# bifurcationkit/BifurcationKit.jl

Hardware: NVIDIA H100
Metric: continuation steps/sec (SH2d PALC) (higher is better)
Workload: dtype f64

## Files before the change

### bifurcationkit.jl_b200/csrc/bk_common.cuh

```cuda
#pragma once
#include <cuda_runtime.h>
#include <stdint.h>
#include <stdlib.h>
#include <string>
#include <unordered_map>
#include <vector>
#include "../../include/bk200.h"
#include <nvtx3/nvToolsExt.h>

struct BkRange {
  explicit BkRange(const char* name) { nvtxRangePushA(name); }
  ~BkRange() { nvtxRangePop(); }
};

#define BK_MAX_PAR 8
#define BK_NSM_FALLBACK 132

struct OpDesc {
  int kind;
  int nx, ny, nz;
  double cx, cy, cz;
  double par[BK_MAX_PAR];
  const double* u;
  double a0, a1;
  long long N;
  int bordered;
  const double* ba;
  const double* bb;
  double bc, bshift, bscale;
  const double* ba2;
  const double* bb2;
  double bc01, bc10, bc11;
  const double* phi;
  const double* fcache;
  int cplx;
  double a0i;
  int transpose;
};

namespace bkg {
#define BKG_MAXPASS 16
struct Plan {
  int n;
  int L;
  int npass;
  int radix[BKG_MAXPASS];
  const double2* wl;
  const double2* ph;
  double dst_scale;
};
}

enum { PW_NONE = 0, PW_RESID = 1, PW_JVP = 2, PW_FLEFT = 3, PW_FRIGHT = 4 };
struct PerPw {
  int pro;
  int epi;
  const double* v;
  const double* u;
  const double* sp;
  double a0, a1, l, nu;
  double spc;
};
#define PW_D 1

struct Precond {
  int kind = BK_PC_NONE;
  double a0 = 0, a1 = 0;
  double* lam[3] = {nullptr, nullptr, nullptr};
  int ttype[3] = {0, 0, 0};
  int fast[3] = {0, 0, 0};
  double2* ftw[3] = {nullptr, nullptr, nullptr};
  double2* fom[3] = {nullptr, nullptr, nullptr};
  double2* flam2[3] = {nullptr, nullptr, nullptr};
  bkg::Plan gplan[3] = {};
  double2* gwl[3] = {nullptr, nullptr, nullptr};
  double2* gph[3] = {nullptr, nullptr, nullptr};
  double* work = nullptr;
  double* work2 = nullptr;
  double* tri = nullptr;
  double2* tdft = nullptr;
  double po_r = 0, po_nu = 0, po_T = 0;
};

struct BkKindTraits {
  int ndims;
  int fields;
  int extra;
  bool jac_sym;
  bool has_jt;
  bool complex_ok;
  bool pow2_grid;
  bool has_jets;
};
const BkKindTraits* bk_kind_traits(int kind);

struct BkEventTimer {
  std::vector<std::pair<cudaEvent_t, cudaEvent_t>> pairs;
  size_t used = 0;
  void begin(cudaStream_t st) {
    if (used == pairs.size()) {
      cudaEvent_t a, b;
      cudaEventCreate(&a);
      cudaEventCreate(&b);
      pairs.push_back({a, b});
    }
    cudaEventRecord(pairs[used++].first, st);
  }
  void end(cudaStream_t st) { cudaEventRecord(pairs[used - 1].second, st); }
  long long harvest(double& ms) {
    long long k = 0;
    for (size_t i = 0; i < used; ++i) {
      float t = 0;
      if (cudaEventElapsedTime(&t, pairs[i].first, pairs[i].second) == cudaSuccess) {
        ms += t;
        ++k;
      }
    }
    used = 0;
    return k;
  }
  void destroy() {
    for (auto& p : pairs) {
      cudaEventDestroy(p.first);
      cudaEventDestroy(p.second);
    }
    pairs.clear();
    used = 0;
  }
};

struct bk_ctx {
  int device = 0;
  int nsm = BK_NSM_FALLBACK;
  cudaStream_t stream = nullptr;
  int kind = 0;
  long long dims[3] = {1, 1, 1};
  double lengths[3] = {1, 1, 1};
  double par[BK_MAX_PAR] = {0};
  long long N = 0;
  long long N0 = 0;
  bool cplx = false;
  double shift_imag = 0;
  bool transpose = false;
  int m = 0;
  long long ld = 0;
  double* u_state = nullptr;
  double jpar[BK_MAX_PAR] = {0};
  bool have_state = false;
  double* phi = nullptr;
  double* xpi = nullptr;
  double* fcache = nullptr;
  double phi_dot_xpi = 0;
  double* V = nullptr;
  double* w = nullptr;
  double* z = nullptr;
  double* r = nullptr;
  double* scales = nullptr;
  double* gcoef = nullptr;
  double* hcols = nullptr;
  double* hcols2 = nullptr;
  double* h_pinned = nullptr;
  double* partials = nullptr;
  int gmax = 0;
  unsigned int* counters = nullptr;
  double* red_out = nullptr;
  double* red_pinned = nullptr;
  double* coef_pinned = nullptr;
  std::vector<cudaEvent_t> events;
  std::vector<double*> stage;
  double* host_pinned = nullptr;
  std::vector<double*> tmp;
  double* mom_stage = nullptr;
  size_t mom_stage_cap = 0;
  void* mom_work = nullptr;
  size_t mom_work_cap = 0;
  std::unordered_map<double*, size_t> vec_live;
  std::vector<std::pair<size_t, double*>> vec_pool;
  double* Q = nullptr;
  double* Q2 = nullptr;
  int q2cap = 0;
  int qcap = 0;
  double* eig_dev = nullptr;
  double* eig_pinned = nullptr;
  Precond pc;
  bk_stats stats = {};
  bool timing = false;
  int timing_every = 1;
  long long solve_count = 0;
  bool timing_now = false;
  BkEventTimer fused_timer;
  BkEventTimer pc_timer;
  std::unordered_map<const void*, size_t> smem_attr;
  std::string err;
};

int bk_fail(bk_ctx* c, int code, const char* what, const char* file, int line);
#define BK_CUDA(c, expr)                                                             \
  do {                                                                               \
    cudaError_t _e = (expr);                                                         \
    if (_e != cudaSuccess) return bk_fail((c), BK_ERR_CUDA, cudaGetErrorString(_e), __FILE__, __LINE__); \
  } while (0)
#define BK_CHECK(c, cond, msg)                                                       \
  do {                                                                               \
    if (!(cond)) return bk_fail((c), BK_ERR_ARG, (msg), __FILE__, __LINE__);         \
  } while (0)
#define BK_ENTER(c)                                 \
  do {                                              \
    if (!(c)) return BK_ERR_ARG;                    \
    if (cudaSetDevice((c)->device) != cudaSuccess)  \
      return bk_fail((c), BK_ERR_CUDA, "cudaSetDevice failed", __FILE__, __LINE__); \
  } while (0)
#define BK_TRY(expr)                 \
  do {                               \
    int _s = (expr);                 \
    if (_s < 0) return _s;           \
  } while (0)

static inline int bk_lin_grid(const bk_ctx* c, long long n) {
  long long g = (n + 255) / 256;
  long long cap = (long long)c->nsm * 8;
  return (int)(g < cap ? (g > 0 ? g : 1) : cap);
}
static inline int bk_reduce_grid(const bk_ctx* c, long long n) {
  const int g = bk_lin_grid(c, n);
  return g < c->gmax ? g : c->gmax;
}
static inline double bk_inv_h2(const bk_ctx* c, int d) {
  const double h = 2 * c->lengths[d] / c->dims[d];
  return 1.0 / (h * h);
}

bool bk_is_device_ptr(const void* p);
int bk_stage_in(bk_ctx* c, const double* p, long long n, int slot, bool copy_in, double** dev);
int bk_stage_out(bk_ctx* c, double* p, long long n, const double* dev);

OpDesc bk_make_op(bk_ctx* c, double a0, double a1);
OpDesc bk_make_residual_op(bk_ctx* c);
int bk_launch_residual(bk_ctx* c, const double* u_dev, double* out_dev);
int bk_launch_apply(bk_ctx* c, const OpDesc& op, const double* in_dev, const double* in_scale_ptr, double* out_dev);
int bk_potrap_refresh_cache(bk_ctx* c);

int bk_precond_apply_dev(bk_ctx* c, const double* in_dev, double* out_dev, long long n);

int bk_periodic_setup(bk_ctx* c);
int bk_periodic_residual(bk_ctx* c, const OpDesc& op, const double* u, double* out);
int bk_periodic_jvp(bk_ctx* c, const OpDesc& op, const double* in, const double* sp, double* out);
int bk_periodic_fused(bk_ctx* c, const OpDesc& op, const double* in, const double* sp, double* out, bool left);

int bk_dev_axpby(bk_ctx* c, double* y, double a, const double* x, double b, long long n);
int bk_dev_scale(bk_ctx* c, double* x, double a, long long n);
int bk_dev_dot(bk_ctx* c, const double* x, const double* y, long long n, double* out_host);
int bk_dev_norminf(bk_ctx* c, const double* x, long long n, double* out_host);
int bk_dev_copy(bk_ctx* c, double* dst, const double* src, long long n);

int bk_gmres_dev(bk_ctx* c, const OpDesc& op, const double* rhs_dev, double* x_dev, const bk_gmres_opts* o,
                 int* converged, int* iters, double* resnorm);
int bk_launch_dots(bk_ctx* c, const double* basis, const double* scales, const double* w, long long n, int j, double* hcol,
                   double* gcoef);
int bk_launch_update(bk_ctx* c, const double* basis, const double* gcoef, const double* w, long long n, int j, double* vout,
                     double* h_out, double* scale_out);
int bk_launch_lincomb(bk_ctx* c, const double* basis, const double* scales, double* x, double beta, long long n, int k,
                      const double* coef_dev);
int bk_tmp(bk_ctx* c, int slot, double** out);

void bk_grant_smem(int device, const void* kern, size_t bytes);
template <typename K>
static inline void bk_ensure_smem(bk_ctx* c, K kern, size_t bytes) {
  size_t& cur = c->smem_attr[(const void*)kern];
  if (bytes > cur) {
    bk_grant_smem(c->device, (const void*)kern, bytes);
    cur = bytes;
  }
}

#ifdef __CUDACC__
template <typename... KArgs, typename... Args>
static inline cudaError_t bk_launch_pdl(void (*kern)(KArgs...), dim3 grid, dim3 block, size_t smem, cudaStream_t st, bool pdl,
                                        Args&&... args) {
  cudaLaunchConfig_t cfg = {};
  cfg.gridDim = grid;
  cfg.blockDim = block;
  cfg.dynamicSmemBytes = smem;
  cfg.stream = st;
  cudaLaunchAttribute at[1];
  at[0].id = cudaLaunchAttributeProgrammaticStreamSerialization;
  at[0].val.programmaticStreamSerializationAllowed = 1;
  cfg.attrs = at;
  static int no_pdl = -1;
  if (no_pdl < 0) no_pdl = getenv("BK_NO_PDL") ? 1 : 0;
  cfg.numAttrs = pdl && !no_pdl ? 1 : 0;
  return cudaLaunchKernelEx(&cfg, kern, KArgs(args)...);
}
template <typename... KArgs, typename... Args>
static inline int bk_launch_ex(bk_ctx* c, bool pdl, void (*kern)(KArgs...), dim3 grid, dim3 block, size_t smem,
                               Args&&... args) {
  if (smem) bk_ensure_smem(c, kern, smem);
  bk_launch_pdl(kern, grid, block, smem, c->stream, pdl, static_cast<Args&&>(args)...);
  BK_CUDA(c, cudaGetLastError());
  c->stats.kernel_launches++;
  return BK_OK;
}
template <typename... KArgs, typename... Args>
static inline int bk_launch(bk_ctx* c, void (*kern)(KArgs...), dim3 grid, dim3 block, size_t smem, Args&&... args) {
  return bk_launch_ex(c, true, kern, grid, block, smem, static_cast<Args&&>(args)...);
}
template <typename... KArgs, typename... Args>
static inline int bk_launch_ordered(bk_ctx* c, void (*kern)(KArgs...), dim3 grid, dim3 block, size_t smem, Args&&... args) {
  return bk_launch_ex(c, false, kern, grid, block, smem, static_cast<Args&&>(args)...);
}
__device__ __forceinline__ void bk_pdl_sync() {
  asm volatile("griddepcontrol.wait;" ::: "memory");
  asm volatile("griddepcontrol.launch_dependents;" ::: "memory");
}
#endif

#ifdef __CUDACC__
__device__ __forceinline__ double bk_warp_sum(double v) {
#pragma unroll
  for (int o = 16; o > 0; o >>= 1) v += __shfl_xor_sync(0xffffffffu, v, o);
  return v;
}
__device__ __forceinline__ double bk_nanmax(double a, double b) { return (a != a) ? a : ((b != b) ? b : fmax(a, b)); }
__device__ __forceinline__ double bk_warp_max(double v) {
#pragma unroll
  for (int o = 16; o > 0; o >>= 1) v = bk_nanmax(v, __shfl_xor_sync(0xffffffffu, v, o));
  return v;
}
__device__ __forceinline__ bool bk_last_block(unsigned int* counter, int* s_flag) {
  __threadfence();
  __syncthreads();
  if (threadIdx.x == 0) {
    unsigned int t = atomicAdd(counter, 1u);
    int last = (t == gridDim.x * gridDim.y * gridDim.z - 1);
    if (last) *counter = 0u;
    *s_flag = last;
  }
  __syncthreads();
  bool last = (*s_flag != 0);
  if (last) __threadfence();
  return last;
}
template <bool MAX>
__device__ __forceinline__ double bk_red(double a, double b) { return MAX ? bk_nanmax(a, b) : a + b; }
template <int K, bool MAX = false>
__device__ __forceinline__ bool bk_grid_reduce(double (&v)[K], double* __restrict__ partials, unsigned int* counter) {
  __shared__ double s_w[K][8];
  __shared__ int s_flag;
  const int lane = threadIdx.x & 31, wid = threadIdx.x >> 5;
#pragma unroll
  for (int k = 0; k < K; ++k) {
    const double t = MAX ? bk_warp_max(v[k]) : bk_warp_sum(v[k]);
    if (lane == 0) s_w[k][wid] = t;
  }
  __syncthreads();
  if (threadIdx.x < K) {
    double t = 0.0;
    for (int w = 0; w < 8; ++w) t = bk_red<MAX>(t, s_w[threadIdx.x][w]);
    partials[(size_t)threadIdx.x * gridDim.x + blockIdx.x] = t;
  }
  if (!bk_last_block(counter, &s_flag)) return false;
  double t[K];
#pragma unroll
  for (int k = 0; k < K; ++k) t[k] = 0.0;
  for (int i = threadIdx.x; i < (int)gridDim.x; i += blockDim.x)
#pragma unroll
    for (int k = 0; k < K; ++k) t[k] = bk_red<MAX>(t[k], __ldcg(partials + (size_t)k * gridDim.x + i));
#pragma unroll
  for (int k = 0; k < K; ++k) {
    t[k] = MAX ? bk_warp_max(t[k]) : bk_warp_sum(t[k]);
    if (lane == 0) s_w[k][wid] = t[k];
  }
  __syncthreads();
  if (threadIdx.x != 0) return false;
#pragma unroll
  for (int k = 0; k < K; ++k) {
    v[k] = 0.0;
    for (int w = 0; w < 8; ++w) v[k] = bk_red<MAX>(v[k], s_w[k][w]);
  }
  return true;
}
#endif
```

### bifurcationkit.jl_b200/csrc/bk_precond.cu

```cuda
#include <cmath>
#include <cstdlib>
#include <utility>
#include <vector>
#include "bk_common.cuh"

#include "bk_fft_fast.cuh"
#include "bk_fft_gen.cuh"

static __global__ void __launch_bounds__(256) k_sh_symbol_div(double* __restrict__ a, int nx, int ny, int nz,
                                                              const double* __restrict__ lx, const double* __restrict__ ly,
                                                              const double* __restrict__ lz, double shift, double scale) {
  const long long total = (long long)nx * ny * nz;
  for (long long q = (long long)blockIdx.x * blockDim.x + threadIdx.x; q < total; q += (long long)gridDim.x * blockDim.x) {
    int i = (int)(q % nx), j = (int)((q / nx) % ny), k = (int)(q / ((long long)nx * ny));
    double t = 1.0 + lx[i] + ly[j] + (lz ? lz[k] : 0.0);
    a[q] = a[q] * scale / (t * t + shift);
  }
}
static __global__ void __launch_bounds__(256) k_helmholtz_symbol_div(double* __restrict__ a, int nx, int ny, long long nblocks,
                                                                     const double* __restrict__ lx,
                                                                     const double* __restrict__ ly, double a0, double a1) {
  const long long n = (long long)nx * ny, total = n * nblocks;
  for (long long q = (long long)blockIdx.x * blockDim.x + threadIdx.x; q < total; q += (long long)gridDim.x * blockDim.x) {
    long long g = q % n;
    int i = (int)(g % nx), j = (int)(g / nx);
    a[q] = a[q] / (a0 + a1 * (lx[i] + ly[j]));
  }
}

#define BK_PO_KMAX 64
static __global__ void __launch_bounds__(128) k_potrap_time(double* __restrict__ B, long long n, int nx, int K,
                                                            const double* __restrict__ lamx, const double* __restrict__ lamy,
                                                            double h, double r, double nu, const double2* __restrict__ tw) {
  const long long g = (long long)blockIdx.x * blockDim.x + threadIdx.x;
  if (g >= n) return;
  const double lam = lamx[g % nx] + lamy[g / nx];
  double2 wp[BK_PO_KMAX], wm[BK_PO_KMAX];
  for (int i = 0; i < K; ++i) {
    const double a = B[(long long)(2 * i) * n + g], b = B[(long long)(2 * i + 1) * n + g];
    wp[i] = make_double2(a, b);
    wm[i] = make_double2(a, -b);
  }
  double2 yp[BK_PO_KMAX], ym[BK_PO_KMAX];
  const double invK = 1.0 / K;
  for (int k = 0; k < K; ++k) {
    double2 ap = make_double2(0, 0), am = make_double2(0, 0);
    int idx = 0;
    for (int i = 0; i < K; ++i) {
      const double2 t = tw[idx];
      ap.x += wp[i].x * t.x - wp[i].y * t.y;
      ap.y += wp[i].x * t.y + wp[i].y * t.x;
      am.x += wm[i].x * t.x - wm[i].y * t.y;
      am.y += wm[i].x * t.y + wm[i].y * t.x;
      idx += k;
      if (idx >= K) idx -= K;
    }
    const double2 gk = tw[k];
    const double2 omg = make_double2(1.0 - gk.x, -gk.y), opg = make_double2(1.0 + gk.x, gk.y);
    const double cr = lam + r;
    double2 sp = make_double2(omg.x - 0.5 * h * (opg.x * cr - opg.y * nu), omg.y - 0.5 * h * (opg.x * nu + opg.y * cr));
    double2 sm = make_double2(omg.x - 0.5 * h * (opg.x * cr + opg.y * nu), omg.y - 0.5 * h * (-opg.x * nu + opg.y * cr));
    const double dp = 1.0 / (sp.x * sp.x + sp.y * sp.y), dm = 1.0 / (sm.x * sm.x + sm.y * sm.y);
    yp[k] = make_double2((ap.x * sp.x + ap.y * sp.y) * dp * invK, (ap.y * sp.x - ap.x * sp.y) * dp * invK);
    ym[k] = make_double2((am.x * sm.x + am.y * sm.y) * dm * invK, (am.y * sm.x - am.x * sm.y) * dm * invK);
  }
  for (int i = 0; i < K; ++i) {
    double2 ap = make_double2(0, 0), am = make_double2(0, 0);
    int idx = 0;
    for (int k = 0; k < K; ++k) {
      const double2 t = tw[idx];
      ap.x += yp[k].x * t.x + yp[k].y * t.y;
      ap.y += yp[k].y * t.x - yp[k].x * t.y;
      am.x += ym[k].x * t.x + ym[k].y * t.y;
      am.y += ym[k].y * t.x - ym[k].x * t.y;
      idx += i;
      if (idx >= K) idx -= K;
    }
    B[(long long)(2 * i) * n + g] = 0.5 * (ap.x + am.x);
    B[(long long)(2 * i + 1) * n + g] = 0.5 * (ap.y - am.y);
  }
}
static __global__ void __launch_bounds__(128) k_potrap_time_tr(double* __restrict__ B, long long n, int nx, int K,
                                                               const double* __restrict__ lamx, const double* __restrict__ lamy,
                                                               double h, double r, double nu, const double2* __restrict__ tw) {
  const long long g = (long long)blockIdx.x * blockDim.x + threadIdx.x;
  if (g >= n) return;
  const double lam = lamx[g % nx] + lamy[g / nx];
  double2 wp[BK_PO_KMAX], wm[BK_PO_KMAX];
  for (int i = 0; i < K; ++i) {
    double a = B[(long long)(2 * i) * n + g], b = B[(long long)(2 * i + 1) * n + g];
    if (i == 0) {
      a += B[(long long)(2 * K) * n + g];
      b += B[(long long)(2 * K + 1) * n + g];
    }
    wp[i] = make_double2(a, b);
    wm[i] = make_double2(a, -b);
  }
  double2 yp[BK_PO_KMAX], ym[BK_PO_KMAX];
  const double invK = 1.0 / K;
  for (int k = 0; k < K; ++k) {
    double2 ap = make_double2(0, 0), am = make_double2(0, 0);
    int idx = 0;
    for (int i = 0; i < K; ++i) {
      const double2 t = tw[idx];
      ap.x += wp[i].x * t.x - wp[i].y * t.y;
      ap.y += wp[i].x * t.y + wp[i].y * t.x;
      am.x += wm[i].x * t.x - wm[i].y * t.y;
      am.y += wm[i].x * t.y + wm[i].y * t.x;
      idx += k;
      if (idx >= K) idx -= K;
    }
    const double2 gk = tw[k];
    const double2 omg = make_double2(1.0 - gk.x, -gk.y), opg = make_double2(1.0 + gk.x, gk.y);
    const double cr = lam + r;
    double2 sp = make_double2(omg.x - 0.5 * h * (opg.x * cr - opg.y * nu), omg.y - 0.5 * h * (opg.x * nu + opg.y * cr));
    double2 sm = make_double2(omg.x - 0.5 * h * (opg.x * cr + opg.y * nu), omg.y - 0.5 * h * (-opg.x * nu + opg.y * cr));
    sp.y = -sp.y;
    sm.y = -sm.y;
    const double dp = 1.0 / (sp.x * sp.x + sp.y * sp.y), dm = 1.0 / (sm.x * sm.x + sm.y * sm.y);
    yp[k] = make_double2((ap.x * sp.x + ap.y * sp.y) * dp * invK, (ap.y * sp.x - ap.x * sp.y) * dp * invK);
    ym[k] = make_double2((am.x * sm.x + am.y * sm.y) * dm * invK, (am.y * sm.x - am.x * sm.y) * dm * invK);
  }
  for (int i = 0; i < K; ++i) {
    double2 ap = make_double2(0, 0), am = make_double2(0, 0);
    int idx = 0;
    for (int k = 0; k < K; ++k) {
      const double2 t = tw[idx];
      ap.x += yp[k].x * t.x + yp[k].y * t.y;
      ap.y += yp[k].y * t.x - yp[k].x * t.y;
      am.x += ym[k].x * t.x + ym[k].y * t.y;
      am.y += ym[k].y * t.x - ym[k].x * t.y;
      idx += i;
      if (idx >= K) idx -= K;
    }
    B[(long long)(2 * i) * n + g] = 0.5 * (ap.x + am.x);
    B[(long long)(2 * i + 1) * n + g] = 0.5 * (ap.y - am.y);
  }
}
static __global__ void __launch_bounds__(256) k_potrap_close(const double* __restrict__ in, double* __restrict__ out,
                                                             long long Ns, int M) {
  const long long i = (long long)blockIdx.x * blockDim.x + threadIdx.x;
  if (i < Ns) out[(long long)(M - 1) * Ns + i] = in[(long long)(M - 1) * Ns + i] + out[i];
  if (i == 0) out[(long long)M * Ns] = in[(long long)M * Ns];
}

static __global__ void k_thomas(const double* __restrict__ tri, const double* __restrict__ in, double* __restrict__ out, int n) {
  if (blockIdx.x != 0 || threadIdx.x != 0) return;
  const double* cp = tri;
  const double* di = tri + n;
  const double* lo = tri + 2 * n;
  double prev = in[0] * di[0];
  out[0] = prev;
  for (int i = 1; i < n; ++i) {
    prev = (in[i] - lo[i] * prev) * di[i];
    out[i] = prev;
  }
  for (int i = n - 2; i >= 0; --i) out[i] -= cp[i] * out[i + 1];
}

static int upload(bk_ctx* c, void** dst, const void* src, size_t bytes) {
  if (*dst) cudaFree(*dst);
  *dst = nullptr;
  BK_CUDA(c, cudaMalloc(dst, bytes));
  BK_CUDA(c, cudaMemcpy(*dst, src, bytes, cudaMemcpyHostToDevice));
  return BK_OK;
}

static int fast_loge(long long n) {
  static int e = -1;
  if (e < 0) {
    const char* a = getenv("BK_FFT_LOGE");
    e = a ? atoi(a) : 0;
    if (e < 2 || e > 5) e = 0;
  }
  if (e) return e;
  return n >= 1024 ? 3 : 2;
}
static int fast_logn(long long n) {
  static int off = -1;
  if (off < 0) off = getenv("BK_FFT_NO_FAST") ? 1 : 0;
  if (off) return 0;
  for (int l = fast_loge(n) + 1; l <= 11; ++l)
    if (l >= 6 && n == (1LL << l)) return l;
  return 0;
}
#define BKF_DISPATCH_N(LE, LOGN, ...)                                                   \
  switch (LOGN) {                                                                      \
    case 6: { using FC = bkf::Cfg<6, LE>; __VA_ARGS__; } break;                        \
    case 7: { using FC = bkf::Cfg<7, LE>; __VA_ARGS__; } break;                        \
    case 8: { using FC = bkf::Cfg<8, LE>; __VA_ARGS__; } break;                        \
    case 9: { using FC = bkf::Cfg<9, LE>; __VA_ARGS__; } break;                        \
    case 10: { using FC = bkf::Cfg<10, LE>; __VA_ARGS__; } break;                      \
    default: { using FC = bkf::Cfg<11, LE>; __VA_ARGS__; } break;                      \
  }
#define BKF_DISPATCH(LOGN, ...)                                                        \
  switch (fast_loge(1LL << (LOGN))) {                                                               \
    case 2: BKF_DISPATCH_N(2, LOGN, __VA_ARGS__) break;                                \
    case 3: BKF_DISPATCH_N(3, LOGN, __VA_ARGS__) break;                                \
    case 4: BKF_DISPATCH_N(4, LOGN, __VA_ARGS__) break;                                \
    default: BKF_DISPATCH_N(5, LOGN, __VA_ARGS__) break;                               \
  }

template <class FC>
static int fast_setup(bk_ctx* c, int d, const double* lam_host) {
  std::vector<double> tw, om, lam2;
  bkf::build_tables<FC>(tw, om, lam2, lam_host);
  Precond& pc = c->pc;
  if (tw.empty()) tw.assign(2, 0.0);
  BK_TRY(upload(c, (void**)&pc.ftw[d], tw.data(), 8 * tw.size()));
  BK_TRY(upload(c, (void**)&pc.fom[d], om.data(), 8 * om.size()));
  BK_TRY(upload(c, (void**)&pc.flam2[d], lam2.data(), 8 * lam2.size()));
  return BK_OK;
}

template <class FC>
static int fast_launch(bk_ctx* c, int d, bool strided, int mode, const double* in, double* out, const bkf::Geom& g,
                       const bkf::Symbol* sy, const PerPw* pw = nullptr) {
  Precond& pc = c->pc;
  bkf::Tables tb{pc.ftw[d], pc.fom[d], pc.flam2[d]};
  bkf::Symbol s0{};
  if (sy) s0 = *sy;
  PerPw p0{};
  if (pw) p0 = *pw;
  if (strided) {
    static decltype(&bkf::k_strided<FC, 0>) const kern[4] = {bkf::k_strided<FC, 0>, bkf::k_strided<FC, 1>, bkf::k_strided<FC, 2>,
                                                             bkf::k_strided<FC, 3>};
    const dim3 grid((g.nb + 2 * FC::PP - 1) / (2 * FC::PP), g.nouter);
    return bk_launch(c, kern[mode], grid, dim3(FC::THREADS), mode >= 2 ? FC::SMEM_FUSED : FC::SMEM, in, out, g, tb, s0);
  }
  static decltype(&bkf::k_contig<FC, 0>) const kern[4] = {bkf::k_contig<FC, 0>, bkf::k_contig<FC, 1>, bkf::k_contig<FC, 2>,
                                                          bkf::k_contig<FC, 3>};
  const dim3 grid((unsigned)((g.nb + 2 * FC::PP - 1) / (2 * FC::PP)));
  return bk_launch(c, kern[mode], grid, dim3(FC::THREADS), FC::SMEM, in, out, g, tb, p0);
}

static void factorize(int L, bkg::Plan& pl) {
  pl.npass = 0;
  while (L % 4 == 0 && pl.npass < BKG_MAXPASS) {
    pl.radix[pl.npass++] = 4;
    L /= 4;
  }
  for (int p = 2; L > 1 && pl.npass < BKG_MAXPASS; ++p)
    while (L % p == 0 && pl.npass < BKG_MAXPASS) {
      pl.radix[pl.npass++] = p;
      L /= p;
    }
}
#define BKG_THREADS 512
#define BKG_SMEM_BUDGET (100 * 1024)
#define BKG_SMEM_MAX (200 * 1024)
static int gen_ppg(int L) {
  long long per = 32LL * L;
  int p = (int)(BKG_SMEM_BUDGET / per);
  if (p < 1) p = 1;
  if (p > 8) p = 8;
  return p;
}

static int gen_setup(bk_ctx* c, int d, int n, int type) {
  Precond& pc = c->pc;
  bkg::Plan& pl = pc.gplan[d];
  pl.n = n;
  pl.L = type == 0 ? 2 * n : 2 * n + 2;
  BK_CHECK(c, 32LL * pl.L <= BKG_SMEM_MAX, "line too long for the general transform kernel (n <= 3199)");
  factorize(pl.L, pl);
  const long double PI = 3.14159265358979323846264338327950288L;
  std::vector<double> wl(2 * (size_t)pl.L), ph(2 * (size_t)n);
  for (int t = 0; t < pl.L; ++t) {
    wl[2 * t] = (double)cosl(-2.0L * PI * t / pl.L);
    wl[2 * t + 1] = (double)sinl(-2.0L * PI * t / pl.L);
  }
  for (int k = 0; k < n; ++k) {
    ph[2 * k] = (double)cosl(-PI * k / (2.0L * n));
    ph[2 * k + 1] = (double)sinl(-PI * k / (2.0L * n));
  }
  BK_TRY(upload(c, (void**)&pc.gwl[d], wl.data(), 8 * wl.size()));
  BK_TRY(upload(c, (void**)&pc.gph[d], ph.data(), 8 * ph.size()));
  pl.wl = pc.gwl[d];
  pl.ph = pc.gph[d];
  pl.dst_scale = 0.5 * sqrt(2.0 / (n + 1.0));
  return BK_OK;
}

static int gen_launch(bk_ctx* c, int d, bool strided, int mode, const double* in, double* out, const bkf::Geom& g) {
  const bkg::Plan& pl = c->pc.gplan[d];
  const int ppg = gen_ppg(pl.L);
  const size_t sm = 32 * (size_t)pl.L * ppg;
  const long long npairs = ((long long)g.nb + 1) / 2;
  dim3 grid((unsigned)((npairs + ppg - 1) / ppg), strided ? g.nouter : 1);
  static decltype(&bkg::k_gen<false, 0>) const kern[2][3] = {{bkg::k_gen<false, 0>, bkg::k_gen<false, 1>, bkg::k_gen<false, 2>},
                                                              {bkg::k_gen<true, 0>, bkg::k_gen<true, 1>, bkg::k_gen<true, 2>}};
  return bk_launch(c, kern[strided][mode], grid, dim3(BKG_THREADS), sm, in, out, g, pl, ppg);
}

static int setup_dim(bk_ctx* c, int d, long long n, double inv_h2, int type, bool even_nx) {
  Precond& pc = c->pc;
  std::vector<double> lam(n);
  const long double PI = 3.14159265358979323846264338327950288L;
  for (long long k = 0; k < n; ++k)
    lam[k] = (type == 0) ? (double)((2.0L * cosl(PI * k / n) - 2.0L)) * inv_h2
                         : (double)(-(2.0L - 2.0L * cosl(PI * (k + 1) / (n + 1)))) * inv_h2;
  BK_TRY(upload(c, (void**)&pc.lam[d], lam.data(), 8 * n));
  pc.ttype[d] = type;
  pc.fast[d] = (type == 0 && even_nx) ? fast_logn(n) : 0;
  if (pc.fast[d]) {
    BKF_DISPATCH(pc.fast[d], BK_TRY(fast_setup<FC>(c, d, lam.data())));
  }
  return gen_setup(c, d, (int)n, type);
}

int bk_periodic_setup(bk_ctx* c) {
  Precond& pc = c->pc;
  const long double PI = 3.14159265358979323846264338327950288L;
  for (int d = 0; d < 2; ++d) {
    const long long n = c->dims[d];
    int logn = 0;
    while ((1LL << logn) < n) ++logn;
    std::vector<double> lam(n);
    for (long long k = 0; k < n; ++k) {
      const long double ks = (long double)(k <= n / 2 ? k : k - n), w = PI * ks / (long double)c->lengths[d];
      lam[k] = (double)(-w * w);
    }
    BK_TRY(upload(c, (void**)&pc.lam[d], lam.data(), 8 * n));
    pc.fast[d] = logn;
    BKF_DISPATCH(logn, BK_TRY(fast_setup<FC>(c, d, lam.data())));
  }
  if (!pc.work) BK_CUDA(c, cudaMalloc(&pc.work, 8 * (size_t)c->ld));
  if (!pc.work2) BK_CUDA(c, cudaMalloc(&pc.work2, 8 * (size_t)c->ld));
  return BK_OK;
}

static int periodic_pipeline(bk_ctx* c, const double* in, double* out, const PerPw& pw, bool neg, double gain, double shift,
                             const double* tail_src = nullptr, double* tail_dst = nullptr, int tail_n = 0) {
  Precond& pc = c->pc;
  const int nx = (int)c->dims[0], ny = (int)c->dims[1];
  const bkf::Geom gx{1, nx, ny, 1}, gy{nx, (long long)nx * ny, nx, 1};
  const bkf::Symbol sy{pc.lam[0], nullptr, shift, gain / ((double)nx * (double)ny), tail_src, tail_dst, tail_n, neg ? 1 : 0};
  BKF_DISPATCH(pc.fast[0], BK_TRY(fast_launch<FC>(c, 0, false, 2, in, pc.work, gx, nullptr, &pw)));
  BKF_DISPATCH(pc.fast[1], BK_TRY(fast_launch<FC>(c, 1, true, 3, pc.work, pc.work2, gy, &sy)));
  BKF_DISPATCH(pc.fast[0], BK_TRY(fast_launch<FC>(c, 0, false, 3, pc.work2, out, gx, nullptr, &pw)));
  return BK_OK;
}

int bk_periodic_residual(bk_ctx* c, const OpDesc& op, const double* u, double* out) {
  const PerPw pw{0, PW_RESID, u, nullptr, nullptr, 0.0, 0.0, op.par[0], op.par[1], 0.0};
  return periodic_pipeline(c, u, out, pw, true, 1.0, 0.0);
}
int bk_periodic_jvp(bk_ctx* c, const OpDesc& op, const double* in, const double* sp, double* out) {
  const PerPw pw{0, PW_JVP, in, op.u, sp, op.a0, op.a1, op.par[0], op.par[1], 0.0};
  return periodic_pipeline(c, in, out, pw, true, op.a1, 0.0);
}
int bk_periodic_fused(bk_ctx* c, const OpDesc& op, const double* in, const double* sp, double* out, bool left) {
  BK_CHECK(c, c->pc.kind == BK_PC_SH_FFT && !op.bordered && !op.cplx, "internal: one-transform operator needs BK_PC_SH_FFT, unbordered, real");
  const PerPw pw{left ? PW_D : 0, left ? PW_FLEFT : PW_FRIGHT, in, op.u, sp, op.a0, op.a1, op.par[0], op.par[1], c->pc.a0};
  return periodic_pipeline(c, in, out, pw, false, 1.0, c->pc.a0);
}

extern "C" int32_t bk_precond_setup(bk_ctx* c, int32_t kind, double a0, double a1) {
  BK_ENTER(c);
  BK_CUDA(c, cudaStreamSynchronize(c->stream));
  Precond& pc = c->pc;
  if (kind == BK_PC_NONE) {
    pc.kind = BK_PC_NONE;
    return BK_OK;
  }
  if (!pc.work) BK_CUDA(c, cudaMalloc(&pc.work, 8 * (size_t)c->ld));
  if (!pc.work2) BK_CUDA(c, cudaMalloc(&pc.work2, 8 * (size_t)c->ld));
  const bool even_nx = (c->dims[0] % 2) == 0;
  if (kind == BK_PC_SH_DCT) {
    BK_CHECK(c, c->kind == BK_SH2D || c->kind == BK_SH3D, "BK_PC_SH_DCT needs a Swift-Hohenberg context");
    for (int d = 0; d < bk_kind_traits(c->kind)->ndims; ++d) BK_TRY(setup_dim(c, d, c->dims[d], bk_inv_h2(c, d), 0, even_nx));
  } else if (kind == BK_PC_SH_FFT) {
    BK_CHECK(c, c->kind == BK_SH2D_PERIODIC, "BK_PC_SH_FFT needs a BK_SH2D_PERIODIC context");
    BK_CHECK(c, a0 > 0, "BK_PC_SH_FFT: a0 must be > 0 (the symbol of L1 vanishes at |k| = 1)");
  } else if (kind == BK_PC_CGL_DST) {
    BK_CHECK(c, c->kind == BK_CGL2D || c->kind == BK_POTRAP_CGL2D, "BK_PC_CGL_DST needs a cGL context");
    for (int d = 0; d < 2; ++d) BK_TRY(setup_dim(c, d, c->dims[d], bk_inv_h2(c, d), 1, even_nx));
  } else if (kind == BK_PC_POTRAP_CIRC) {
    BK_CHECK(c, c->kind == BK_POTRAP_CGL2D, "BK_PC_POTRAP_CIRC needs a Trapeze (potrap) context");
    const int K = (int)c->dims[2] - 1;
    BK_CHECK(c, K >= 1 && K <= BK_PO_KMAX, "BK_PC_POTRAP_CIRC supports 2 <= M <= 65 time slices");
    BK_CHECK(c, a0 > 0, "BK_PC_POTRAP_CIRC: a0 must be the period T > 0");
    for (int d = 0; d < 2; ++d) BK_TRY(setup_dim(c, d, c->dims[d], bk_inv_h2(c, d), 1, even_nx));
    std::vector<double2> tw(K);
    const long double PI = 3.14159265358979323846264338327950288L;
    for (int j = 0; j < K; ++j) tw[j] = make_double2((double)cosl(-2.0L * PI * j / K), (double)sinl(-2.0L * PI * j / K));
    BK_TRY(upload(c, (void**)&pc.tdft, tw.data(), 16 * (size_t)K));
    pc.po_T = a0;
    pc.po_r = c->par[0];
    pc.po_nu = c->par[2];
  } else if (kind == BK_PC_CHAN_TRIDIAG) {
    BK_CHECK(c, c->kind == BK_CHAN, "BK_PC_CHAN_TRIDIAG needs a chan context");
    long long n = c->N0;
    double s = (double)(n - 1) * (double)(n - 1);
    std::vector<double> lo(n, s), di(n, -2 * s), up(n, s), tri(3 * n);
    di[0] = 1;
    up[0] = 0;
    lo[n - 1] = 0;
    di[n - 1] = 1;
    lo[0] = 0;
    up[n - 1] = 0;
    double denom = di[0];
    tri[n + 0] = 1.0 / denom;
    tri[0] = up[0] / denom;
    for (long long i = 1; i < n; ++i) {
      denom = di[i] - lo[i] * tri[i - 1];
      tri[n + i] = 1.0 / denom;
      tri[i] = up[i] / denom;
      tri[2 * n + i] = lo[i];
    }
    BK_TRY(upload(c, (void**)&pc.tri, tri.data(), 8 * 3 * n));
  } else {
    return bk_fail(c, BK_ERR_ARG, "unknown preconditioner kind", __FILE__, __LINE__);
  }
  pc.kind = kind;
  pc.a0 = a0;
  pc.a1 = a1;
  return BK_OK;
}

static int transform_pass(bk_ctx* c, int d, int mode, const double* in, double* out, int nx, int ny, int nz, bool aligned,
                          const bkf::Symbol* fused = nullptr) {
  Precond& pc = c->pc;
  bkf::Geom g;
  bool strided = d != 0;
  if (d == 0) {
    g.es = 1;
    g.os = nx;
    g.nb = ny * nz;
    g.nouter = 1;
  } else if (d == 1) {
    g.es = nx;
    g.nb = nx;
    g.os = (long long)nx * ny;
    g.nouter = nz;
  } else {
    g.es = (long long)nx * ny;
    g.nb = nx;
    g.os = nx;
    g.nouter = ny;
  }
  if (pc.fast[d] && aligned) {
    BKF_DISPATCH(pc.fast[d], BK_TRY(fast_launch<FC>(c, d, strided, fused ? 2 : mode, in, out, g, fused)));
  } else {
    BK_CHECK(c, !fused, "internal: fused transform on the general path");
    BK_TRY(gen_launch(c, d, strided, pc.ttype[d] == 1 ? 2 : mode, in, out, g));
  }
  return BK_OK;
}

static inline bool aligned16(const void* a, const void* b) { return ((((uintptr_t)a) | ((uintptr_t)b)) & 15) == 0; }

static int precond_apply_one(bk_ctx* c, const double* in, double* out, long long n);

int bk_precond_apply_dev(bk_ctx* c, const double* in, double* out, long long n) {
  BK_CHECK(c, c->pc.kind != BK_PC_NONE, "no preconditioner set up (bk_precond_setup)");
  BK_CHECK(c, in != out, "preconditioner: in-place application is not supported");
  if (!c->cplx) return precond_apply_one(c, in, out, n);
  BK_CHECK(c, n >= c->N, "preconditioner: vector shorter than the complexified problem");
  BK_TRY(precond_apply_one(c, in, out, c->N0));
  return precond_apply_one(c, in + c->N0, out + c->N0, n - c->N0);
}

static int precond_apply_one(bk_ctx* c, const double* in, double* out, long long n) {
  Precond& pc = c->pc;
  const long long N = c->N0;
  bool tail_done = false;
  const bool timed = c->timing_now;
  if (timed) c->pc_timer.begin(c->stream);
  const bool al = aligned16(in, out);
  if (pc.kind == BK_PC_SH_DCT) {
    const int nd = bk_kind_traits(c->kind)->ndims;
    const int nx = (int)c->dims[0], ny = (int)c->dims[1], nz = nd == 3 ? (int)c->dims[2] : 1;
    double* A = pc.work;
    double* B = pc.work2;
    const int last = nd - 1;
    double scale = 1.0;
    for (int d = 0; d < nd; ++d) scale /= 2.0 * (double)c->dims[d];
    if (pc.fast[last] && al) {
      bkf::Symbol sy{pc.lam[0], nd == 3 ? pc.lam[1] : nullptr, pc.a0, scale, nullptr, nullptr, 0};
      if (n > N && n - N <= 32) {
        sy.tail_src = in + N;
        sy.tail_dst = out + N;
        sy.tail_n = (int)(n - N);
        tail_done = true;
      }
      BK_TRY(transform_pass(c, 0, 0, in, A, nx, ny, nz, al));
      if (nd == 3) {
        BK_TRY(transform_pass(c, 1, 0, A, B, nx, ny, nz, true));
        BK_TRY(transform_pass(c, 2, 0, B, A, nx, ny, nz, true, &sy));
        BK_TRY(transform_pass(c, 1, 1, A, B, nx, ny, nz, true));
        BK_TRY(transform_pass(c, 0, 1, B, out, nx, ny, nz, al));
      } else {
        BK_TRY(transform_pass(c, 1, 0, A, B, nx, ny, nz, true, &sy));
        BK_TRY(transform_pass(c, 0, 1, B, out, nx, ny, nz, al));
      }
    } else {
      BK_TRY(transform_pass(c, 0, 0, in, A, nx, ny, nz, al));
      BK_TRY(transform_pass(c, 1, 0, A, B, nx, ny, nz, true));
      double* cur = B;
      double* oth = A;
      if (nd == 3) {
        BK_TRY(transform_pass(c, 2, 0, B, A, nx, ny, nz, true));
        cur = A;
        oth = B;
      }
      BK_TRY(bk_launch_ordered(c, k_sh_symbol_div, bk_lin_grid(c, N), 256, 0, cur, nx, ny, nz, pc.lam[0], pc.lam[1],
                               nd == 3 ? pc.lam[2] : nullptr, pc.a0, scale));
      if (nd == 3) {
        BK_TRY(transform_pass(c, 2, 1, cur, oth, nx, ny, nz, true));
        std::swap(cur, oth);
      }
      BK_TRY(transform_pass(c, 1, 1, cur, oth, nx, ny, nz, true));
      BK_TRY(transform_pass(c, 0, 1, oth, out, nx, ny, nz, al));
    }
  } else if (pc.kind == BK_PC_SH_FFT) {
    const double* ts = nullptr;
    double* td = nullptr;
    int tn = 0;
    if (n > N && n - N <= 32) {
      ts = in + N;
      td = out + N;
      tn = (int)(n - N);
      tail_done = true;
    }
    const PerPw pw{0, PW_NONE, in, nullptr, nullptr, 0.0, 0.0, 0.0, 0.0, 0.0};
    BK_TRY(periodic_pipeline(c, in, out, pw, false, 1.0, pc.a0, ts, td, tn));
  } else if (pc.kind == BK_PC_CGL_DST) {
    const int nx = (int)c->dims[0], ny = (int)c->dims[1];
    const long long nblk = (c->kind == BK_POTRAP_CGL2D) ? 2 * c->dims[2] : 2;
    double* A = pc.work;
    double* B = pc.work2;
    BK_TRY(transform_pass(c, 0, 0, in, A, nx, ny, (int)nblk, al));
    BK_TRY(transform_pass(c, 1, 0, A, B, nx, ny, (int)nblk, true));
    BK_TRY(bk_launch_ordered(c, k_helmholtz_symbol_div, bk_lin_grid(c, (long long)nx * ny * nblk), 256, 0, B, nx, ny, nblk,
                             pc.lam[0], pc.lam[1], pc.a0, pc.a1));
    BK_TRY(transform_pass(c, 1, 1, B, A, nx, ny, (int)nblk, true));
    BK_TRY(transform_pass(c, 0, 1, A, out, nx, ny, (int)nblk, al));
    if (c->kind == BK_POTRAP_CGL2D) BK_CUDA(c, cudaMemcpyAsync(out + N - 1, in + N - 1, 8, cudaMemcpyDeviceToDevice, c->stream));
  } else if (pc.kind == BK_PC_POTRAP_CIRC) {
    const int nx = (int)c->dims[0], ny = (int)c->dims[1], M = (int)c->dims[2];
    const long long nn = (long long)nx * ny, Ns = 2 * nn;
    const int nf = 2 * M;
    double* A = pc.work;
    double* Bf = pc.work2;
    BK_TRY(transform_pass(c, 0, 0, in, A, nx, ny, nf, al));
    BK_TRY(transform_pass(c, 1, 0, A, Bf, nx, ny, nf, true));
    BK_TRY(bk_launch_ordered(c, c->transpose ? k_potrap_time_tr : k_potrap_time, (unsigned)((nn + 127) / 128), 128, 0, Bf, nn, nx,
                             M - 1, pc.lam[0], pc.lam[1], pc.po_T / M, pc.po_r, pc.po_nu, pc.tdft));
    BK_TRY(transform_pass(c, 1, 1, Bf, A, nx, ny, nf, true));
    BK_TRY(transform_pass(c, 0, 1, A, out, nx, ny, nf, al));
    if (c->transpose)
      BK_CUDA(c, cudaMemcpyAsync(out + (M - 1) * Ns, in + (M - 1) * Ns, 8 * (size_t)(Ns + 1), cudaMemcpyDeviceToDevice, c->stream));
    else
      BK_TRY(bk_launch_ordered(c, k_potrap_close, (unsigned)((Ns + 255) / 256), 256, 0, in, out, Ns, M));
  } else if (pc.kind == BK_PC_CHAN_TRIDIAG) {
    BK_TRY(bk_launch_ordered(c, k_thomas, 1, 32, 0, pc.tri, in, out, (int)N));
  }
  if (n > N && !tail_done)
    BK_CUDA(c, cudaMemcpyAsync(out + N, in + N, 8 * (size_t)(n - N), cudaMemcpyDeviceToDevice, c->stream));
  if (timed) c->pc_timer.end(c->stream);
  return BK_OK;
}

extern "C" int32_t bk_precond_apply(bk_ctx* c, const double* in, double* out) {
  BK_ENTER(c);
  BkRange nvtx_range("bk_precond_apply");
  double *din, *dout;
  BK_TRY(bk_stage_in(c, in, c->N, 10, true, &din));
  BK_TRY(bk_stage_in(c, out, c->N, 11, false, &dout));
  BK_TRY(bk_precond_apply_dev(c, din, dout, c->N));
  return bk_stage_out(c, out, c->N, dout);
}
```

Measured before the change: 4.376.

## Add persistent TMA-pipelined DCT kernels for the 2D Swift-Hohenberg preconditioner

Adds persistent-grid versions of the contiguous and strided fast DCT kernels, sized from occupancy queries. The contiguous kernel double-buffers rows through bulk async copies and mbarriers, so the load of the next unit overlaps compute on the current one and stores go out as bulk copies. The point is to hide global-memory latency and spread the table staging cost over many units instead of repeating it per block. The path is on by default for 2D with fast transforms and can be turned off with BK_PC_PIPE=0. It adds shared memory per CTA and more synchronisation, which may lower occupancy.

```diff
diff --git a/bifurcationkit.jl_b200/csrc/bk_common.cuh b/bifurcationkit.jl_b200/csrc/bk_common.cuh
--- a/bifurcationkit.jl_b200/csrc/bk_common.cuh
+++ b/bifurcationkit.jl_b200/csrc/bk_common.cuh
@@ -75,6 +75,8 @@
   bkg::Plan gplan[3] = {};
   double2* gwl[3] = {nullptr, nullptr, nullptr};
   double2* gph[3] = {nullptr, nullptr, nullptr};
+  bool pipe = false;
+  int pipe_ctas[3] = {0, 0, 0};
   double* work = nullptr;
   double* work2 = nullptr;
   double* tri = nullptr;
diff --git a/bifurcationkit.jl_b200/csrc/bk_fft_pipe.cuh b/bifurcationkit.jl_b200/csrc/bk_fft_pipe.cuh
--- /dev/null
+++ b/bifurcationkit.jl_b200/csrc/bk_fft_pipe.cuh
@@ -0,0 +1,188 @@
+#pragma once
+#include "bk_fft_fast.cuh"
+
+namespace bkf {
+
+template <class C>
+struct Pipe {
+  static constexpr size_t SMEM_X = C::SMEM + sizeof(double) * 2 * C::PP * C::N;
+  static constexpr size_t SMEM_Y = C::SMEM_FUSED;
+  static constexpr int MINB = C::THREADS <= 256 ? 2 : 1;
+  static_assert(C::SLOTS >= C::N, "work array smaller than the unit's rows");
+};
+
+#ifdef __CUDACC__
+__device__ __forceinline__ void pipe_range(int units, int& u0, int& u1) {
+  u0 = (int)((long long)blockIdx.x * units / gridDim.x);
+  u1 = (int)((long long)(blockIdx.x + 1) * units / gridDim.x);
+}
+template <class C>
+__device__ __forceinline__ void pipe_rows_in(const double* in, const Geom& g, int u, double* stg, unsigned long long* bar) {
+  const long long l0 = (long long)u * 2 * C::PP;
+  const int nv = (int)min((long long)2 * C::PP, (long long)g.nb - l0);
+  constexpr unsigned rb = 8u * C::N;
+  mbar_arrive_expect_tx(bar, rb * nv);
+  for (int l = 0; l < nv; ++l) bulk_g2s(stg + (size_t)l * C::N, in + (l0 + l) * g.os, rb, bar);
+}
+template <class C>
+__device__ __forceinline__ void pipe_rows_out(double* out, const Geom& g, int u, const double* rows) {
+  const long long l0 = (long long)u * 2 * C::PP;
+  const int nv = (int)min((long long)2 * C::PP, (long long)g.nb - l0);
+  for (int l = 0; l < nv; ++l) bulk_s2g(out + (l0 + l) * g.os, rows + (size_t)l * C::N, 8u * C::N);
+  bulk_store_commit();
+}
+
+template <class C, int MODE>
+static __global__ void __launch_bounds__(C::THREADS, Pipe<C>::MINB) k_contig_pipe(const double* __restrict__ in, double* __restrict__ out, Geom g,
+                                                                      Tables tbg) {
+  extern __shared__ __align__(128) double2 sm_fast[];
+  __shared__ __align__(8) unsigned long long tbar, ibar;
+  double2* sm = sm_fast;
+  double* stg = reinterpret_cast<double*>(reinterpret_cast<char*>(sm_fast) + C::SMEM);
+  double* rows = reinterpret_cast<double*>(sm_fast);
+  const Tables tb = stage_tables<C, false>(tbg, sm, &tbar);
+  const int tid = threadIdx.x, pr = tid % C::PP, tau = tid / C::PP;
+  int u0, u1;
+  pipe_range((g.nb + 2 * C::PP - 1) / (2 * C::PP), u0, u1);
+  if (tid == 0) {
+    mbar_init(&ibar, 1);
+    fence_mbar_init();
+  }
+  __syncthreads();
+  bk_pdl_sync();
+  if (tid == 0 && u0 < u1) pipe_rows_in<C>(in, g, u0, stg, &ibar);
+  for (int u = u0, it = 0; u < u1; ++u, ++it) {
+    const long long lineA = ((long long)u * C::PP + pr) * 2, lineB = lineA + 1;
+    const bool vA = lineA < g.nb, vB = lineB < g.nb;
+    const double* sA = stg + (size_t)(2 * pr) * C::N;
+    const double* sB = sA + C::N;
+    double* rA = rows + (size_t)(2 * pr) * C::N;
+    double* rB = rA + C::N;
+    double2 a[C::E];
+    mbar_wait(&ibar, it & 1);
+    if (MODE == 0) {
+#pragma unroll
+      for (int i = 0; i < C::E; ++i) {
+        const int e = row_of<C>(i, tau);
+        a[i] = make_double2(vA ? sA[e] : 0.0, vB ? sB[e] : 0.0);
+      }
+      fence_proxy_async_smem();
+      if (tid == 0) bulk_store_wait_read();
+      __syncthreads();
+      if (tid == 0 && u + 1 < u1) pipe_rows_in<C>(in, g, u + 1, stg, &ibar);
+      if (it == 0) mbar_wait(&tbar, 0);
+      fwd_passes<C, 0>(a, sm, tb, tau, pr);
+      park<C>(a, sm, tau, pr);
+      __syncthreads();
+#pragma unroll
+      for (int reg = 0; reg < C::E; ++reg) {
+        int k;
+        const double2 z = a[reg], zp = partner<C>(sm, reg_pos<C>(tau, reg), pr, k);
+        const double2 w = tb.om[reg * C::T + tau];
+        const double sx = z.x + zp.x, sy_ = z.y - zp.y, dx = z.x - zp.x, dy = z.y + zp.y;
+        a[reg] = make_double2(fma(w.x, sx, -(w.y * sy_)), fma(w.x, dy, w.y * dx));
+      }
+      __syncthreads();
+#pragma unroll
+      for (int reg = 0; reg < C::E; ++reg) sm[nslot<C>(k_of_pos<C>(reg_pos<C>(tau, reg)), pr)] = a[reg];
+      __syncthreads();
+#pragma unroll
+      for (int i = 0; i < C::E; ++i) a[i] = sm[nslot<C>(i * C::T + tau, pr)];
+      __syncthreads();
+#pragma unroll
+      for (int i = 0; i < C::E; ++i) {
+        const int k = i * C::T + tau;
+        rA[k] = a[i].x;
+        rB[k] = a[i].y;
+      }
+    } else {
+      if (tid == 0) bulk_store_wait_read();
+      __syncthreads();
+#pragma unroll
+      for (int i = 0; i < C::E; ++i) {
+        const int k = i * C::T + tau;
+        sm[nslot<C>(k, pr)] = make_double2(vA ? sA[k] : 0.0, vB ? sB[k] : 0.0);
+      }
+      fence_proxy_async_smem();
+      __syncthreads();
+      if (tid == 0 && u + 1 < u1) pipe_rows_in<C>(in, g, u + 1, stg, &ibar);
+      if (it == 0) mbar_wait(&tbar, 0);
+#pragma unroll
+      for (int reg = 0; reg < C::E; ++reg) {
+        const int k = k_of_pos<C>(reg_pos<C>(tau, reg)), nk = (C::N - k) & (C::N - 1);
+        const double2 w = tb.om[reg * C::T + tau];
+        const double2 d = sm[nslot<C>(k, pr)];
+        double2 dn = sm[nslot<C>(nk, pr)];
+        if (k == 0) dn = make_double2(0.0, 0.0);
+        a[reg] = cmulc(make_double2(d.x + dn.y, d.y - dn.x), w);
+      }
+      __syncthreads();
+      inv_passes<C, C::NP - 1>(a, sm, tb, tau, pr);
+      __syncthreads();
+#pragma unroll
+      for (int i = 0; i < C::E; ++i) {
+        const int e = row_of<C>(i, tau);
+        rA[e] = a[i].x;
+        rB[e] = a[i].y;
+      }
+    }
+    fence_proxy_async_smem();
+    __syncthreads();
+    if (tid == 0) pipe_rows_out<C>(out, g, u, rows);
+  }
+  if (tid == 0) bulk_store_wait_all();
+}
+
+template <class C>
+static __global__ void __launch_bounds__(C::THREADS, Pipe<C>::MINB) k_strided_pipe(const double* __restrict__ in, double* __restrict__ out, Geom g,
+                                                                       Tables tbg, Symbol sy) {
+  extern __shared__ __align__(128) double2 sm_fast[];
+  __shared__ __align__(8) unsigned long long tbar;
+  double2* sm = sm_fast;
+  const Tables tb = stage_tables<C, true>(tbg, sm, &tbar);
+  const int tid = threadIdx.x, pr = tid % C::PP, tau = tid / C::PP;
+  int u0, u1;
+  pipe_range((g.nb + 2 * C::PP - 1) / (2 * C::PP), u0, u1);
+  __syncthreads();
+  bk_pdl_sync();
+  if (sy.tail_n > 0 && blockIdx.x == 0 && tid < sy.tail_n) sy.tail_dst[tid] = sy.tail_src[tid];
+  for (int u = u0, it = 0; u < u1; ++u, ++it) {
+    const int col = (u * C::PP + pr) * 2;
+    const bool v0 = col < g.nb, v1 = col + 1 < g.nb;
+    double2 a[C::E];
+    strided_load<C>(a, in + col, g.es, tau, v0, v1);
+    if (it == 0) mbar_wait(&tbar, 0);
+    else __syncthreads();
+    fwd_passes<C, 0>(a, sm, tb, tau, pr);
+    park<C>(a, sm, tau, pr);
+    __syncthreads();
+    const double lo = sy.lam_o ? __ldg(sy.lam_o) : 0.0;
+    const double cA = 1.0 + lo + (v0 ? __ldg(sy.lam_b + col) : 0.0), cB = 1.0 + lo + (v1 ? __ldg(sy.lam_b + col + 1) : 0.0);
+#pragma unroll
+    for (int reg = 0; reg < C::E; ++reg) {
+      int k;
+      const double2 z = a[reg], zp = partner<C>(sm, reg_pos<C>(tau, reg), pr, k);
+      const double2 w = tb.om[reg * C::T + tau];
+      const double2 l2 = tb.lam2[reg * C::T + tau];
+      const double2 A1 = cmul(make_double2(z.x + zp.x, z.y - zp.y), w);
+      const double2 A2 = cmul(make_double2(z.y + zp.y, zp.x - z.x), w);
+      double t = cA + l2.x;
+      const double s1k = fma(t, t, sy.shift);
+      t = cA + l2.y;
+      const double s1n = fma(t, t, sy.shift);
+      t = cB + l2.x;
+      const double s2k = fma(t, t, sy.shift);
+      t = cB + l2.y;
+      const double s2n = fma(t, t, sy.shift);
+      const double r1 = sy.scale * __drcp_rn(s1k * s1n), r2 = sy.scale * __drcp_rn(s2k * s2n);
+      const double h1x = A1.x * (r1 * s1n), h1y = A1.y * (r1 * s1k);
+      const double h2x = A2.x * (r2 * s2n), h2y = A2.y * (r2 * s2k);
+      a[reg] = cmulc(make_double2(h1x - h2y, h1y + h2x), w);
+    }
+    __syncthreads();
+    inv_passes<C, C::NP - 1>(a, sm, tb, tau, pr);
+    strided_store<C>(a, out + col, g.es, tau, v0, v1);
+  }
+}
+#endif
+}
diff --git a/bifurcationkit.jl_b200/csrc/bk_precond.cu b/bifurcationkit.jl_b200/csrc/bk_precond.cu
--- a/bifurcationkit.jl_b200/csrc/bk_precond.cu
+++ b/bifurcationkit.jl_b200/csrc/bk_precond.cu
@@ -5,6 +5,7 @@
 #include "bk_common.cuh"
 
 #include "bk_fft_fast.cuh"
+#include "bk_fft_pipe.cuh"
 #include "bk_fft_gen.cuh"
 
 static __global__ void __launch_bounds__(256) k_sh_symbol_div(double* __restrict__ a, int nx, int ny, int nz,
@@ -166,6 +167,7 @@
   return BK_OK;
 }
 
+static int default_loge(long long n) { return n >= 1024 ? 3 : 2; }
 static int fast_loge(long long n) {
   static int e = -1;
   if (e < 0) {
@@ -174,7 +176,7 @@
     if (e < 2 || e > 5) e = 0;
   }
   if (e) return e;
-  return n >= 1024 ? 3 : 2;
+  return default_loge(n);
 }
 static int fast_logn(long long n) {
   static int off = -1;
@@ -234,6 +236,66 @@
   return bk_launch(c, kern[mode], grid, dim3(FC::THREADS), FC::SMEM, in, out, g, tb, p0);
 }
 
+#define BKF_PIPE_DISPATCH(LOGN, ...)                                                   \
+  switch (LOGN) {                                                                      \
+    case 6: { using FC = bkf::Cfg<6, 2>; __VA_ARGS__; } break;                         \
+    case 7: { using FC = bkf::Cfg<7, 2>; __VA_ARGS__; } break;                         \
+    case 8: { using FC = bkf::Cfg<8, 2>; __VA_ARGS__; } break;                         \
+    case 9: { using FC = bkf::Cfg<9, 2>; __VA_ARGS__; } break;                         \
+    case 10: { using FC = bkf::Cfg<10, 3>; __VA_ARGS__; } break;                       \
+    default: { using FC = bkf::Cfg<11, 3>; __VA_ARGS__; } break;                       \
+  }
+template <class K>
+static int pipe_ctas(bk_ctx* c, K kern, int threads, size_t smem, int* ctas) {
+  bk_ensure_smem(c, kern, smem);
+  int occ = 0;
+  BK_CUDA(c, cudaOccupancyMaxActiveBlocksPerMultiprocessor(&occ, kern, threads, smem));
+  *ctas = c->nsm * occ;
+  return BK_OK;
+}
+template <class FC>
+static int pipe_setup_x(bk_ctx* c) {
+  Precond& pc = c->pc;
+  BK_TRY(pipe_ctas(c, bkf::k_contig_pipe<FC, 0>, FC::THREADS, bkf::Pipe<FC>::SMEM_X, &pc.pipe_ctas[0]));
+  return pipe_ctas(c, bkf::k_contig_pipe<FC, 1>, FC::THREADS, bkf::Pipe<FC>::SMEM_X, &pc.pipe_ctas[2]);
+}
+template <class FC>
+static int pipe_setup_y(bk_ctx* c) {
+  return pipe_ctas(c, bkf::k_strided_pipe<FC>, FC::THREADS, bkf::Pipe<FC>::SMEM_Y, &c->pc.pipe_ctas[1]);
+}
+static int pipe_grid(int ctas, int nb, int pp) {
+  const int units = (nb + 2 * pp - 1) / (2 * pp);
+  return units < ctas ? units : ctas;
+}
+template <class FC>
+static int pipe_launch_x(bk_ctx* c, int mode, const double* in, double* out, const bkf::Geom& g) {
+  Precond& pc = c->pc;
+  const bkf::Tables tb{pc.ftw[0], pc.fom[0], pc.flam2[0]};
+  const int grid = pipe_grid(pc.pipe_ctas[mode == 0 ? 0 : 2], g.nb, FC::PP);
+  return bk_launch(c, mode == 0 ? bkf::k_contig_pipe<FC, 0> : bkf::k_contig_pipe<FC, 1>, dim3(grid), dim3(FC::THREADS),
+                   bkf::Pipe<FC>::SMEM_X, in, out, g, tb);
+}
+template <class FC>
+static int pipe_launch_y(bk_ctx* c, const double* in, double* out, const bkf::Geom& g, const bkf::Symbol& sy) {
+  Precond& pc = c->pc;
+  const bkf::Tables tb{pc.ftw[1], pc.fom[1], pc.flam2[1]};
+  return bk_launch(c, bkf::k_strided_pipe<FC>, dim3(pipe_grid(pc.pipe_ctas[1], g.nb, FC::PP)), dim3(FC::THREADS),
+                   bkf::Pipe<FC>::SMEM_Y, in, out, g, tb, sy);
+}
+static bool pipe_allowed() {
+  const char* a = getenv("BK_PC_PIPE");
+  return !(a && atoi(a) == 0);
+}
+static int pipe_apply(bk_ctx* c, const double* in, double* out, const bkf::Symbol& sy) {
+  Precond& pc = c->pc;
+  const int nx = (int)c->dims[0], ny = (int)c->dims[1];
+  const bkf::Geom gx{1, nx, ny, 1}, gy{nx, (long long)nx * ny, nx, 1};
+  BKF_PIPE_DISPATCH(pc.fast[0], BK_TRY(pipe_launch_x<FC>(c, 0, in, pc.work, gx)));
+  BKF_PIPE_DISPATCH(pc.fast[1], BK_TRY(pipe_launch_y<FC>(c, pc.work, pc.work2, gy, sy)));
+  BKF_PIPE_DISPATCH(pc.fast[0], BK_TRY(pipe_launch_x<FC>(c, 1, pc.work2, out, gx)));
+  return BK_OK;
+}
+
 static void factorize(int L, bkg::Plan& pl) {
   pl.npass = 0;
   while (L % 4 == 0 && pl.npass < BKG_MAXPASS) {
@@ -369,7 +431,15 @@
   const bool even_nx = (c->dims[0] % 2) == 0;
   if (kind == BK_PC_SH_DCT) {
     BK_CHECK(c, c->kind == BK_SH2D || c->kind == BK_SH3D, "BK_PC_SH_DCT needs a Swift-Hohenberg context");
-    for (int d = 0; d < bk_kind_traits(c->kind)->ndims; ++d) BK_TRY(setup_dim(c, d, c->dims[d], bk_inv_h2(c, d), 0, even_nx));
+    const int nd = bk_kind_traits(c->kind)->ndims;
+    for (int d = 0; d < nd; ++d) BK_TRY(setup_dim(c, d, c->dims[d], bk_inv_h2(c, d), 0, even_nx));
+    pc.pipe = false;
+    if (nd == 2 && pc.fast[0] && pc.fast[1] && fast_loge(c->dims[0]) == default_loge(c->dims[0]) &&
+        fast_loge(c->dims[1]) == default_loge(c->dims[1]) && pipe_allowed()) {
+      BKF_PIPE_DISPATCH(pc.fast[0], BK_TRY(pipe_setup_x<FC>(c)));
+      BKF_PIPE_DISPATCH(pc.fast[1], BK_TRY(pipe_setup_y<FC>(c)));
+      pc.pipe = pc.pipe_ctas[0] > 0 && pc.pipe_ctas[1] > 0 && pc.pipe_ctas[2] > 0;
+    }
   } else if (kind == BK_PC_SH_FFT) {
     BK_CHECK(c, c->kind == BK_SH2D_PERIODIC, "BK_PC_SH_FFT needs a BK_SH2D_PERIODIC context");
     BK_CHECK(c, a0 > 0, "BK_PC_SH_FFT: a0 must be > 0 (the symbol of L1 vanishes at |k| = 1)");
@@ -485,13 +555,16 @@
         sy.tail_n = (int)(n - N);
         tail_done = true;
       }
-      BK_TRY(transform_pass(c, 0, 0, in, A, nx, ny, nz, al));
-      if (nd == 3) {
+      if (pc.pipe) {
+        BK_TRY(pipe_apply(c, in, out, sy));
+      } else if (nd == 3) {
+        BK_TRY(transform_pass(c, 0, 0, in, A, nx, ny, nz, al));
         BK_TRY(transform_pass(c, 1, 0, A, B, nx, ny, nz, true));
         BK_TRY(transform_pass(c, 2, 0, B, A, nx, ny, nz, true, &sy));
         BK_TRY(transform_pass(c, 1, 1, A, B, nx, ny, nz, true));
         BK_TRY(transform_pass(c, 0, 1, B, out, nx, ny, nz, al));
       } else {
+        BK_TRY(transform_pass(c, 0, 0, in, A, nx, ny, nz, al));
         BK_TRY(transform_pass(c, 1, 0, A, B, nx, ny, nz, true, &sy));
         BK_TRY(transform_pass(c, 0, 1, B, out, nx, ny, nz, al));
       }
```

New measurement: 4.387 (median of 6 runs). Within noise of the previous version (+0.3%).
